# NikolaZubic/2dimageto3dmodel

Measured on NVIDIA H100. Metric: render+loss+GAN images/sec (cfg3: cfg2 render+loss at batch 32 + conv-GAN 256x256 G/D iteration, 1 G : 2 D, Adam), higher is better.
Workload: dtype tf32 (convs) / f32

## Files before the change

2dimageto3dmodel_b200/csrc/b3d_core.cu:

```cuda
#include <atomic>
#include <stdarg.h>
#include <string.h>

#include "b3d_common.cuh"

namespace b3d {
static thread_local char g_err[512] = "";
static thread_local char g_variant[256] = "";
static std::atomic<uint64_t> g_launches{0};

void set_error(const char* fmt, ...) {
    va_list ap;
    va_start(ap, fmt);
    vsnprintf(g_err, sizeof(g_err), fmt, ap);
    va_end(ap);
}
void clear_variant() { g_variant[0] = 0; }
void add_variant(const char* fmt, ...) {
    size_t n = strlen(g_variant);
    if (n + 2 >= sizeof(g_variant)) return;
    if (n) g_variant[n++] = ';';
    va_list ap;
    va_start(ap, fmt);
    vsnprintf(g_variant + n, sizeof(g_variant) - n, fmt, ap);
    va_end(ap);
}
void count_launch(int n) { g_launches.fetch_add((uint64_t)n, std::memory_order_relaxed); }
}

extern "C" {
const char* b3d_last_error(void) { return b3d::g_err; }
const char* b3d_last_variant(void) { return b3d::g_variant; }
int b3d_version(void) { return 420; }
uint64_t b3d_launch_count(void) { return b3d::g_launches.load(std::memory_order_relaxed); }
}
```

2dimageto3dmodel_b200/csrc/tc_conv.cu:

```cuda
#include "tc_common.cuh"

namespace {

constexpr int BM = 128;
constexpr int BK = 32;
constexpr int MMA_K = 8;
constexpr int MAX_TAPS = 25;
constexpr int NTHREADS = 384;

struct ConvParams {
    int N, Hout, Wout, Cout;
    int BW, BH, BI;
    int tiles_x, tiles_y;
    int xbase;
    int ntaps, kslices;
    int sy, sx;
    int dy[MAX_TAPS], dx[MAX_TAPS];
    int wtap[MAX_TAPS];
    int OH, OW, OC, osy, osx;
    float leaky;
    double* stats;
    int fold;
    int fold_y0;
    int mask;
// ... 174 lines not shown
        tc::tma_prefetch_desc(&tmap_w);
        if (p.mask) tc::tma_prefetch_desc(&tmap_m);
        for (int s = 0; s < STAGES; ++s) {
            for (int o = 0; o < OWNERS; ++o) tc::mbar_init(full + o * STAGES + s, 1);
            tc::mbar_init(empty + s, kEmptyArrivals<BN>);
        }
        tc::fence_barrier_init();
    }
    __syncthreads();
    const int KI = p.ntaps / KW * p.kslices;
    const int MS = p.mask ? BN / 32 : 0;
    const int wg = threadIdx.x >> 7;

    if (wg == 0) {
        tc::setmaxnreg_dec<PRODUCER_REGS>();
        if (threadIdx.x == 0) {
            uint32_t git = 0;
            for (int w = blockIdx.x, k = 0; w < work_items; w += gridDim.x, ++k) {
                uint64_t* fb = full + (COOP ? 0 : (k & 1) * STAGES);
                const int cls = w % p.ncls, wq = w / p.ncls, tb = cls * p.ntaps;
                int t = wq % tiles;
                const int c0 = (wq / tiles) * BN;
                const int x0 = p.xbase + (t % p.tiles_x) * p.BW;
                t /= p.tiles_x;
                const int y0 = (t % p.tiles_y) * p.BH, n0 = (t / p.tiles_y) * p.BI;
                for (int it = 0; it < KI; ++it, ++git) {
                    const int s = git % STAGES;
                    tc::mbar_wait(empty + s, ((git / STAGES) & 1) ^ 1);
                    const int tap = it / p.kslices * KW, ks = it % p.kslices;
                    unsigned char* a = base + s * S::STAGE_BYTES;
                    tc::mbar_arrive_expect_tx(fb + s, S::TX_BYTES);
                    if (KW > 1)
                        tc::tma_load_4d(a, &tmap_x, fb + s, ks * BK, x0 + p.dx0, y0 + p.dy[tb + tap], n0);
                    else if (p.fold)
                        tc::tma_load_4d(a, &tmap_x, fb + s, 0, x0 + p.dx[tb + tap], y0 + p.fold_y0 + 4 * ks, n0);
                    else
                        tc::tma_load_4d(a, &tmap_x, fb + s, ks * BK, p.sx * x0 + p.dx[tb + tap], p.sy * y0 + p.dy[tb + tap], n0);
                    tc::tma_load_3d(a + S::A_BYTES, &tmap_w, fb + s, ks * BK, c0, p.wtap[tb + tap]);
                }
                const int mx = p.osx * x0 + p.coox[cls], my = p.osy * y0 + p.cooy[cls];
                for (int m = 0; m < MS; ++m, ++git) {
                    const int s = git % STAGES;
                    tc::mbar_wait(empty + s, ((git / STAGES) & 1) ^ 1);
                    tc::mbar_arrive_expect_tx(fb + s, MASK_BYTES);
                    tc::tma_load_4d(base + s * S::STAGE_BYTES, &tmap_m, fb + s, c0 + mask_chunk_channel(m, G), mx, my, n0);
                }
            }
        }
        return;
    }
    tc::setmaxnreg_inc<CONSUMER_REGS>();

    const int h = wg - 1, tid = threadIdx.x & 127, lane = tid & 31;
    float acc[kBlocks<BN>][BM / 2];
#pragma unroll
    for (int m = 0; m < kBlocks<BN>; ++m)
#pragma unroll
        for (int i = 0; i < BM / 2; ++i) acc[m][i] = 0.f;
    uint32_t git = 0, phase = 0;
    const uint32_t ring = tc::smem_u32(base);
    TileAt at;
    at.lbw = __ffs(p.BW) - 1;
    at.lbwh = at.lbw + __ffs(p.BH) - 1;
    uint64_t* fb = full + (COOP ? 0 : h * STAGES);
    const int cb = COOP ? 128 * h : 0;
    const int cw = (tid >> 5) * 16 + (lane >> 2);
    const int mine = (COOP ? 2 * h : 0) + (tid >> 6);
    for (int k = COOP ? 0 : h;; k += COOP ? 1 : 2) {
        const int w = blockIdx.x + k * gridDim.x;
        if (w >= work_items) break;
        git = (uint32_t)k * (KI + MS);
        const int wq = w / p.ncls, tile = wq % tiles, c0 = (wq / tiles) * BN + cb;
        tile_origin(p, at, tile, w % p.ncls);
        if (KW == 1 && p.fold) mainloop<BN, STAGES, KW, true>(acc, base, fb, empty, KI, git, phase, cb, tid == 0, p.shift);
        else mainloop<BN, STAGES, KW, false>(acc, base, fb, empty, KI, git, phase, cb, tid == 0, p.shift);
        uint32_t neg[kBlocks<BN>][2] = {};
        if (p.mask) {
#pragma unroll
            for (int m = 0; m < kBlocks<BN>; ++m, git += G) {
                uint32_t mstage = 0;
#pragma unroll
                for (int i = 0; i < G; ++i) {
                    const int s = (git + i) % STAGES;
                    tc::mbar_wait(fb + s, (phase >> s) & 1);
                    phase ^= 1u << s;
                    if (i == mine) mstage = ring + s * S::STAGE_BYTES;
                }
                mask_bits<G, STAGES>(neg[m], mstage, cw, lane, empty, git);
            }
        }
#pragma unroll
        for (int m = 0; m < kBlocks<BN>; ++m) {
            if (p.mask) epilogue_block<true>(acc[m], neg[m], p, at, bias, out, c0 + 64 * m, cw, lane);
            else epilogue_block<false>(acc[m], neg[m], p, at, bias, out, c0 + 64 * m, cw, lane);
        }
    }
}

struct WgradParams {
    int N, Hout, Wout, Cout, Cin;
    int BWk, BHk;
    int kx, ky;
    int kh, kw, pad_y, st;
    int xoff;
    int splits;
    int tapmajor;
    int tstep;
};

template <int BN, int STAGES, int NRAW, int T>
struct WSmem {
    static constexpr int DY_BYTES = BM * BK * 4;
    static constexpr int STAGE_BYTES = T * BN * BK * 4;
    static constexpr int WROWS = T == 1 ? 32 : 36;
    static constexpr int RAW_X = (BN / 32) * WROWS * 128;
    static constexpr int RAW_BYTES = (DY_BYTES + RAW_X + 1023) / 1024 * 1024;
    static constexpr int TOTAL = STAGES * STAGE_BYTES + NRAW * RAW_BYTES + 1024 + 256;
};

__host__ __device__ constexpr int wgrad_row_co(int m) { return (m & 35) | ((m & 8) >> 1) | ((m & 16) >> 1) | ((m & 4) << 2); }

__host__ __device__ constexpr int dy_tile_offset(int co, int px) {
    return (co >> 5) * 4096 + px * 128 + ((((co >> 2) & 7) ^ (px & 7)) << 4) + (co & 3) * 4;
}

__host__ __device__ constexpr int xt_chunk(int i) { return (((i & 7) >> 1) ^ ((i >> 4) & 3)) | (((i >> 3) & 1) << 2); }
__host__ __device__ constexpr int xt_src_offset(int i, int px, int wrows) { return ((i >> 6) * wrows + px) * 128 + (i & 7) * 16; }
__host__ __device__ constexpr int xt_dst_offset(int i, int j) {
    return ((i >> 6) * 32 + 4 * (i & 7) + j) * 128 + ((xt_chunk(i) ^ ((4 * (i & 7) + j) & 7)) << 4);
}
template <int BN, int T, int WROWS>
__device__ __forceinline__ void wgrad_transpose(uint32_t src, uint32_t dst, int tid) {
    constexpr int NT = 2 * BN / 128;
    float4 v[NT][T + 3];
#pragma unroll
    for (int n = 0; n < NT; ++n)
#pragma unroll
        for (int u = 0; u < T + 3; ++u) v[n][u] = tc::lds_f32x4(src + xt_src_offset(tid + 128 * n, 4 * xt_chunk(tid + 128 * n) + u, WROWS));
#pragma unroll
    for (int n = 0; n < NT; ++n) {
        const int i = tid + 128 * n;
#pragma unroll
        for (int t = 0; t < T; ++t) {
            const uint32_t d = dst + t * (BN * 128);
            const float4* w = v[n] + t;
            tc::sts_f32x4(d + xt_dst_offset(i, 0), w[0].x, w[1].x, w[2].x, w[3].x);
            tc::sts_f32x4(d + xt_dst_offset(i, 1), w[0].y, w[1].y, w[2].y, w[3].y);
            tc::sts_f32x4(d + xt_dst_offset(i, 2), w[0].z, w[1].z, w[2].z, w[3].z);
            tc::sts_f32x4(d + xt_dst_offset(i, 3), w[0].w, w[1].w, w[2].w, w[3].w);
        }
    }
}

template <int N, int T, int STAGES, int NRAW, int RAW_BYTES, int STAGE_BYTES>
__device__ __forceinline__ void wgrad_consume(float (&acc)[T][N / 2], uint32_t raw_s, uint32_t stage_s, uint64_t* full,
                                              uint64_t* empty, uint64_t* rawfull, uint64_t* rawempty, const int (&aoff)[4],
                                              int first, int step, int KI, int tid, bool zero_first) {
    using Frag = uint32_t[BK / MMA_K][4];
    auto load = [&](Frag& f, int j) {
        const int rb = j % NRAW;
        tc::mbar_wait(rawfull + rb, (j / NRAW) & 1);
#pragma unroll
        for (int k = 0; k < BK / MMA_K; ++k)
#pragma unroll
            for (int e = 0; e < 4; ++e) f[k][e] = tc::lds_u32(raw_s + rb * RAW_BYTES + aoff[e] + k * 1024);
        __syncwarp();
        if ((tid & 31) == 0) tc::mbar_arrive(rawempty + rb);
    };
    auto slice = [&](int j, Frag& f, Frag& g) {
        const int st = j % STAGES;
        tc::mbar_wait(full + st, (j / STAGES) & 1);
        const uint32_t b = stage_s + st * STAGE_BYTES;
        tc::wgmma_fence();
#pragma unroll
        for (int t = 0; t < T; ++t)
#pragma unroll
            for (int k = 0; k < BK / MMA_K; ++k)
                tc::Wgmma<N>::mma_rs(acc[t], f[k], tc::desc_k128(b + t * (N * 128) + k * MMA_K * 4), (zero_first && j == first && k == 0) ? 0u : 1u);
        tc::wgmma_commit();
        tc::wgmma_wait<1>();
#pragma unroll
        for (int k = 0; k < BK / MMA_K; ++k)
#pragma unroll
            for (int e = 0; e < 4; ++e) tc::fence_operand(g[k][e]);
        if (j != first && tid == 0) tc::mbar_arrive(empty + (j - step) % STAGES);
        if (j + step < KI) load(g, j + step);
    };
    Frag f0, f1;
    if (first < KI) load(f0, first);
    for (int j = first; j < KI; j += 2 * step) {
        slice(j, f0, f1);
        if (j + step < KI) slice(j + step, f1, f0);
    }
    tc::wgmma_wait<0>();
#pragma unroll
    for (int k = 0; k < BK / MMA_K; ++k)
#pragma unroll
        for (int e = 0; e < 4; ++e) {
            tc::fence_operand(f0[k][e]);
            tc::fence_operand(f1[k][e]);
        }
#pragma unroll
    for (int t = 0; t < T; ++t)
#pragma unroll
        for (int i = 0; i < N / 2; ++i) tc::fence_operand(acc[t][i]);
    if (first < KI && tid == 0) tc::mbar_arrive(empty + (first + (KI - 1 - first) / step * step) % STAGES);
}

template <int BN, int STAGES, int NRAW, int T>
__global__ void __launch_bounds__(NTHREADS, 1)
wgrad_wgmma_kernel(const __grid_constant__ CUtensorMap tmap_dy, const __grid_constant__ CUtensorMap tmap_x,
                   const WgradParams p, float* __restrict__ dw) {
    using S = WSmem<BN, STAGES, NRAW, T>;
    extern __shared__ unsigned char smem_raw[];
    unsigned char* base = reinterpret_cast<unsigned char*>((reinterpret_cast<uintptr_t>(smem_raw) + 1023) & ~uintptr_t(1023));
    unsigned char* raw = base + STAGES * S::STAGE_BYTES;
    uint64_t* full = reinterpret_cast<uint64_t*>(raw + NRAW * S::RAW_BYTES);
    uint64_t* empty = full + STAGES;
    uint64_t* rawfull = empty + STAGES;
    uint64_t* rawempty = rawfull + NRAW;

    const int co0 = blockIdx.x * BM, ci0 = blockIdx.y * BN;
    const int gpr = p.kw / T;
    const int groups = p.kh * gpr;
    const int grp = blockIdx.z % groups, split = blockIdx.z / groups;
    const int r = grp / gpr, s = grp % gpr;
    const int per_img = p.kx * p.ky;
    const long long ktotal = (long long)p.N * per_img;
    const long long k_lo = ktotal * split / p.splits, k_hi = ktotal * (split + 1) / p.splits;
    const int KI = (int)(k_hi - k_lo);
    const int nact = co0 + 64 < p.Cout ? 2 : 1;

    if (threadIdx.x == 0) {
        tc::tma_prefetch_desc(&tmap_dy);
        tc::tma_prefetch_desc(&tmap_x);
        for (int i = 0; i < STAGES; ++i) {
            tc::mbar_init(full + i, 128);
            tc::mbar_init(empty + i, nact);
        }
        for (int i = 0; i < NRAW; ++i) {
            tc::mbar_init(rawfull + i, 1);
            tc::mbar_init(rawempty + i, 4 * nact);
        }
        tc::fence_barrier_init();
    }
    __syncthreads();
    const int wg = threadIdx.x >> 7, tid = threadIdx.x & 127;

    if (wg == 0) {
        tc::setmaxnreg_dec<80>();
        auto issue = [&](int j) {
            if (tid != 0) return;
            const long long k = k_lo + j;
            const int n = (int)(k / per_img), rem = (int)(k % per_img);
            const int x0 = (rem % p.kx) * p.BWk, y0 = (rem / p.kx) * p.BHk;
            const int rb = j % NRAW;
            unsigned char* dst = raw + rb * S::RAW_BYTES;
            tc::mbar_wait(rawempty + rb, ((j / NRAW) & 1) ^ 1);
            tc::mbar_arrive_expect_tx(rawfull + rb, S::DY_BYTES + S::RAW_X);
            tc::tma_load_5d(dst, &tmap_dy, rawfull + rb, 0, x0, y0, n, co0 / 32);
            tc::tma_load_5d(dst + S::DY_BYTES, &tmap_x, rawfull + rb, 0, p.st * x0 + s + p.xoff, p.st * y0 + r - p.pad_y, n, ci0 / 32);
        };
        for (int j = 0; j < NRAW - 1 && j < KI; ++j) issue(j);
        const uint32_t raw_s = tc::smem_u32(raw), base_s = tc::smem_u32(base);
        for (int it = 0; it < KI; ++it) {
            if (it + NRAW - 1 < KI) issue(it + NRAW - 1);
            const int rb = it % NRAW, st = it % STAGES;
            tc::mbar_wait(rawfull + rb, (it / NRAW) & 1);
            tc::mbar_wait(empty + st, ((it / STAGES) & 1) ^ 1);
            wgrad_transpose<BN, T, S::WROWS>(raw_s + rb * S::RAW_BYTES + S::DY_BYTES, base_s + st * S::STAGE_BYTES, tid);
            tc::fence_proxy_async();
            tc::mbar_arrive(full + st);
            tc::named_sync(2, 128);
        }
        return;
    }
    tc::setmaxnreg_inc<208>();

    const int h = wg - 1, lane = tid & 31;
    if (h >= nact) return;
    int aoff[4];
#pragma unroll
    for (int e = 0; e < 4; ++e)
        aoff[e] = dy_tile_offset(h * 64 + wgrad_row_co((tid >> 5) * 16 + (lane >> 2) + 8 * (e & 1)), (lane & 3) + 4 * (e >> 1));
    float acc[T][BN / 2];
#pragma unroll
    for (int t = 0; t < T; ++t)
#pragma unroll
        for (int i = 0; i < BN / 2; ++i) acc[t][i] = 0.f;
    wgrad_consume<BN, T, STAGES, NRAW, S::RAW_BYTES, S::STAGE_BYTES>(acc, tc::smem_u32(raw), tc::smem_u32(base), full, empty, rawfull,
                                                                     rawempty, aoff, 0, 1, KI, tid, true);
    if (KI == 0) return;
    const int m_a = (tid >> 5) * 16 + (lane >> 2);
    const int cq = ci0 + 2 * (lane & 3);
#pragma unroll
    for (int t = 0; t < T; ++t) {
        const int sc = s + t * p.tstep;
#pragma unroll
        for (int e = 0; e < 2; ++e) {
            const int co = co0 + h * 64 + wgrad_row_co(m_a + 8 * e);
            if (co >= p.Cout) continue;
#pragma unroll
            for (int j = 0; j < BN / 8; ++j) {
                const int ci = cq + 8 * j;
                if (ci >= p.Cin) continue;
                const float v0 = acc[t][4 * j + 2 * e], v1 = acc[t][4 * j + 2 * e + 1];
                if (p.tapmajor) {
                    atomicAdd(reinterpret_cast<float2*>(dw + ((size_t)(r * p.kw + sc) * p.Cout + co) * p.Cin + ci), make_float2(v0, v1));
                } else {
                    atomicAdd(dw + (((size_t)co * p.Cin + ci) * p.kh + r) * p.kw + sc, v0);
                    atomicAdd(dw + (((size_t)co * p.Cin + ci + 1) * p.kh + r) * p.kw + sc, v1);
                }
            }
        }
    }
}

template <int BN, int STAGES, int NRAW, int T>
int launch_wgrad(const CUtensorMap& mdy, const CUtensorMap& mx, const WgradParams& p, float* dw, dim3 grid, cudaStream_t st) {
    using S = WSmem<BN, STAGES, NRAW, T>;
    static_assert(S::TOTAL <= 227 * 1024, "wgrad pipeline does not fit shared memory");
    B3D_CUDA_OK(cudaFuncSetAttribute(wgrad_wgmma_kernel<BN, STAGES, NRAW, T>, cudaFuncAttributeMaxDynamicSharedMemorySize, S::TOTAL));
    wgrad_wgmma_kernel<BN, STAGES, NRAW, T><<<grid, NTHREADS, S::TOTAL, st>>>(mdy, mx, p, dw);
    B3D_LAUNCH_OK();
    b3d::add_variant("wgrad_wgmma<%d,%d,%d,%d>", BN, STAGES, NRAW, T);
    return B3D_OK;
}

constexpr int STEM_KW = 5, STEM_STAGES = 4, STEM_NRAW = 3;
constexpr int STEM_BATCH = 3;
struct StemSmem {
    static constexpr int DY_BYTES = 64 * BK * 4;
    static constexpr int WPX = BK + STEM_KW - 1;
    static constexpr int RAW_X_MAX = 8 * WPX * 32;
    static constexpr int RAW_BYTES = (DY_BYTES + RAW_X_MAX + 1023) / 1024 * 1024;
    static constexpr int TILE_BYTES = 64 * BK * 4;
    static constexpr int STAGE_BYTES = STEM_KW * TILE_BYTES;
    static constexpr int TOTAL = STEM_STAGES * STAGE_BYTES + STEM_NRAW * RAW_BYTES + 1024 + 256;
};

__global__ void __launch_bounds__(NTHREADS, 1)
wgrad_stem_kernel(const __grid_constant__ CUtensorMap tmap_dy, const __grid_constant__ CUtensorMap tmap_x,
                  const WgradParams p, int fold_kh, float* __restrict__ dw) {
    using S = StemSmem;
    extern __shared__ unsigned char smem_raw[];
    unsigned char* base = reinterpret_cast<unsigned char*>((reinterpret_cast<uintptr_t>(smem_raw) + 1023) & ~uintptr_t(1023));
    unsigned char* raw = base + STEM_STAGES * S::STAGE_BYTES;
    uint64_t* full = reinterpret_cast<uint64_t*>(raw + STEM_NRAW * S::RAW_BYTES);
    uint64_t* empty = full + STEM_STAGES;
    uint64_t* rawfull = empty + STEM_STAGES;
    uint64_t* rawempty = rawfull + STEM_NRAW;

    const int co0 = blockIdx.x * 64, split = blockIdx.y;
    const int per_img = p.kx * p.ky;
    const long long ktotal = (long long)p.N * per_img;
    const long long k_lo = ktotal * split / p.splits, k_hi = ktotal * (split + 1) / p.splits;
    const int KI = (int)(k_hi - k_lo);
    const int creal = 8 * fold_kh;
    const int xbytes = fold_kh * S::WPX * 32;

    if (threadIdx.x == 0) {
        tc::tma_prefetch_desc(&tmap_dy);
        tc::tma_prefetch_desc(&tmap_x);
        for (int i = 0; i < STEM_STAGES; ++i) {
            tc::mbar_init(full + i, 128);
            tc::mbar_init(empty + i, 1);
        }
        for (int i = 0; i < STEM_NRAW; ++i) {
            tc::mbar_init(rawfull + i, 1);
            tc::mbar_init(rawempty + i, 4);
        }
        tc::fence_barrier_init();
    }
    __syncthreads();
    const int wg = threadIdx.x >> 7, tid = threadIdx.x & 127;

    if (wg == 0) {
        tc::setmaxnreg_dec<56>();
        auto issue = [&](int j) {
            if (tid != 0) return;
            const long long k = k_lo + j;
            const int n = (int)(k / per_img), rem = (int)(k % per_img);
            const int x0 = (rem % p.kx) * BK, y0 = rem / p.kx;
            const int rb = j % STEM_NRAW;
            unsigned char* dst = raw + rb * S::RAW_BYTES;
            tc::mbar_wait(rawempty + rb, ((j / STEM_NRAW) & 1) ^ 1);
            tc::mbar_arrive_expect_tx(rawfull + rb, S::DY_BYTES + xbytes);
            tc::tma_load_5d(dst, &tmap_dy, rawfull + rb, 0, x0, y0, n, co0 / 32);
            tc::tma_load_4d(dst + S::DY_BYTES, &tmap_x, rawfull + rb, 0, x0, y0 - p.pad_y, n);
        };
        for (int i = tid; i < STEM_STAGES * STEM_KW * (64 - creal) * 8; i += 128) {
            const int c = creal + (i >> 3) % (64 - creal), tile = (i >> 3) / (64 - creal);
            *reinterpret_cast<float4*>(base + tile * S::TILE_BYTES + c * 128 + (i & 7) * 16) = make_float4(0.f, 0.f, 0.f, 0.f);
        }
        for (int j = 0; j < STEM_NRAW - 1 && j < KI; ++j) issue(j);
        const int ntask = fold_kh * 8 * STEM_KW * 8;
        const uint32_t raw_s = tc::smem_u32(raw), base_s = tc::smem_u32(base);
        for (int it = 0; it < KI; ++it) {
            if (it + STEM_NRAW - 1 < KI) issue(it + STEM_NRAW - 1);
            const int rb = it % STEM_NRAW, st = it % STEM_STAGES;
            tc::mbar_wait(rawfull + rb, (it / STEM_NRAW) & 1);
            tc::mbar_wait(empty + st, ((it / STEM_STAGES) & 1) ^ 1);
            const uint32_t src = raw_s + rb * S::RAW_BYTES + S::DY_BYTES;
            const uint32_t dst = base_s + st * S::STAGE_BYTES;
            for (int i0 = tid; i0 < ntask; i0 += STEM_BATCH * 128) {
                float v[STEM_BATCH][4];
                uint32_t d[STEM_BATCH];
#pragma unroll
                for (int g = 0; g < STEM_BATCH; ++g) {
                    const int i = i0 + 128 * g;
                    if (i >= ntask) break;
                    const int ci = i & 7, u = i >> 3;
                    const int s = u % STEM_KW, q = (u / STEM_KW) & 7, r = u / (STEM_KW * 8);
                    const uint32_t a = src + ((r * S::WPX + 4 * q + s) * 8 + ci) * 4;
#pragma unroll
                    for (int e = 0; e < 4; ++e) v[g][e] = tc::lds_f32(a + 32 * e);
                    d[g] = dst + s * S::TILE_BYTES + (8 * r + ci) * 128 + ((q ^ ci) << 4);
                }
#pragma unroll
                for (int g = 0; g < STEM_BATCH; ++g) {
                    if (i0 + 128 * g >= ntask) break;
                    tc::sts_f32x4(d[g], v[g][0], v[g][1], v[g][2], v[g][3]);
                }
            }
            tc::fence_proxy_async();
            tc::mbar_arrive(full + st);
            tc::named_sync(2, 128);
        }
        return;
    }
    tc::setmaxnreg_inc<224>();

    const int h = wg - 1, lane = tid & 31;
    int aoff[4];
#pragma unroll
    for (int e = 0; e < 4; ++e)
        aoff[e] = dy_tile_offset(wgrad_row_co((tid >> 5) * 16 + (lane >> 2) + 8 * (e & 1)), (lane & 3) + 4 * (e >> 1));
    float acc[STEM_KW][32];
#pragma unroll
    for (int t = 0; t < STEM_KW; ++t)
#pragma unroll
        for (int i = 0; i < 32; ++i) acc[t][i] = 0.f;
    static_assert(S::TILE_BYTES == 64 * 128, "a tap's B tile is 64 channel rows of 128 bytes");
    wgrad_consume<64, STEM_KW, STEM_STAGES, STEM_NRAW, S::RAW_BYTES, S::STAGE_BYTES>(acc, tc::smem_u32(raw), tc::smem_u32(base), full, empty,
                                                                                     rawfull, rawempty, aoff, h, 2, KI, tid, false);
    if (h >= KI) return;
    const int m_a = (tid >> 5) * 16 + (lane >> 2);
#pragma unroll
    for (int t = 0; t < STEM_KW; ++t) {
#pragma unroll
        for (int e = 0; e < 2; ++e) {
            const int co = co0 + wgrad_row_co(m_a + 8 * e);
#pragma unroll
            for (int j = 0; j < 8; ++j) {
                const int ci = 8 * j + 2 * (lane & 3);
                if (ci >= creal) continue;
                const float v0 = acc[t][4 * j + 2 * e], v1 = acc[t][4 * j + 2 * e + 1];
                if (p.tapmajor) {
                    atomicAdd(reinterpret_cast<float2*>(dw + ((size_t)t * p.Cout + co) * p.Cin + ci), make_float2(v0, v1));
                } else {
                    atomicAdd(dw + ((size_t)co * p.Cin + ci) * STEM_KW + t, v0);
                    atomicAdd(dw + ((size_t)co * p.Cin + ci + 1) * STEM_KW + t, v1);
                }
            }
        }
    }
}

int wgrad_splits(int base_ctas, long long ktotal) {
    constexpr long long FIXED = 16;
    const long long sms = tc::num_sms();
    long long smax = ktotal / 8;
    if (smax > 8 * sms) smax = 8 * sms;
    int best = 1;
    long long best_cost = -1;
    for (long long s = 1; s <= smax; ++s) {
        const long long cost = (base_ctas * s + sms - 1) / sms * ((ktotal + s - 1) / s + FIXED);
        if (best_cost < 0 || cost < best_cost) { best = (int)s; best_cost = cost; }
    }
    return best;
}

template <int BN, int STAGES, int KW = 1>
int launch_conv(const CUtensorMap& mx, const CUtensorMap& mw, const CUtensorMap& mm, const ConvParams& p, const float* bias, float* out,
                int tiles, cudaStream_t st) {
    using S = CSmem<BN, STAGES, KW>;
    static_assert(S::TOTAL <= 227 * 1024, "conv pipeline does not fit shared memory");
    B3D_CUDA_OK(cudaFuncSetAttribute(conv_wgmma_kernel<BN, STAGES, KW>, cudaFuncAttributeMaxDynamicSharedMemorySize, S::TOTAL));
    const int work = tiles * b3d::ceil_div(p.Cout, BN) * p.ncls;
    const int sms = tc::num_sms();
    conv_wgmma_kernel<BN, STAGES, KW><<<work < sms ? work : sms, NTHREADS, S::TOTAL, st>>>(mx, mw, mm, p, bias, out, tiles, work);
    B3D_LAUNCH_OK();
    if (KW > 1) b3d::add_variant("conv_wgmma_rowwin<%d,%d,%d>", BN, KW, STAGES);
    else b3d::add_variant("conv_wgmma<%d,%d>", BN, STAGES);
    return B3D_OK;
}

template <int BN>
int launch_rowwin(int kw, const CUtensorMap& mx, const CUtensorMap& mw, const CUtensorMap& mm, const ConvParams& p, const float* bias,
                  float* out, int tiles, cudaStream_t st) {
    if (kw == 2) return launch_conv<BN, BN == 64 ? 5 : 4, 2>(mx, mw, mm, p, bias, out, tiles, st);
    if (kw == 3) return launch_conv<BN, BN == 64 ? 4 : 3, 3>(mx, mw, mm, p, bias, out, tiles, st);
    return launch_conv<BN, BN == 64 ? 3 : 2, 5>(mx, mw, mm, p, bias, out, tiles, st);
}

int pow2_floor(int v) {
    int p = 1;
    while (p * 2 <= v) p *= 2;
    return p;
}

}

extern "C" {

int b3d_conv2d_tf32(const float* x, const float* wt, const float* bias, float* out, int N, int H, int W, int Cin,
                    int Hout, int Wout, int Cout, int ntaps, const int* dy, const int* dx, int sy, int sx, int OH,
                    int OW, int OC, int osy, int osx, int ooy, int oox, float leaky, const int* wtap,
                    int wtaps_total, double* stats, int fold_kh, int fold_pad, const b3d_conv_opts* opts, void* stream) {
    B3D_REQUIRE(N > 0 && H > 0 && W > 0 && Hout > 0 && Wout > 0 && Cout > 0, B3D_EINVAL, "b3d_conv2d_tf32: bad sizes");
    B3D_REQUIRE(Cin > 0 && Cin % BK == 0, B3D_EINVAL, "b3d_conv2d_tf32: Cin=%d must be a multiple of %d", Cin, BK);
    B3D_REQUIRE(ntaps >= 1 && ntaps <= MAX_TAPS && dy && dx, B3D_EINVAL, "b3d_conv2d_tf32: bad taps");
    B3D_REQUIRE(x && wt && out, B3D_EINVAL, "b3d_conv2d_tf32: null pointer");
    B3D_REQUIRE(sy >= 1 && sy <= 2 && sx >= 1 && sx <= 2, B3D_EINVAL, "b3d_conv2d_tf32: stride must be 1 or 2");
    if (!wtap) wtaps_total = ntaps;
    B3D_REQUIRE(wtaps_total >= ntaps || wtap, B3D_EINVAL, "b3d_conv2d_tf32: bad weight tap count");
    for (int t = 0; wtap && t < ntaps; ++t)
        B3D_REQUIRE(wtap[t] >= 0 && wtap[t] < wtaps_total, B3D_EINVAL, "b3d_conv2d_tf32: weight tap %d out of range", wtap[t]);
    B3D_CHECK_ALIGNED(x);
    B3D_CHECK_ALIGNED(wt);
    b3d::clear_variant();

    const float* mask = opts ? opts->mask : nullptr;
    const float mslope = opts ? opts->mask_slope : 1.f;
    B3D_REQUIRE(!mask || (reinterpret_cast<uintptr_t>(mask) % 16 == 0 && OC % 4 == 0), B3D_EINVAL,
                "b3d_conv2d_tf32: the mask needs a 16-byte aligned base and OC %% 4 == 0 (OC=%d)", OC);
    const int stats_sum = (opts && opts->stats_sum_only) ? 1 : 0;
    const int xpitch = (opts && opts->x_row_pitch) ? opts->x_row_pitch : W;
    const int ncls = (opts && opts->nclass > 1) ? opts->nclass : 1;
    B3D_REQUIRE(ncls <= 4 && ntaps % ncls == 0 && (ncls == 1 || (sy == 1 && sx == 1 && fold_kh == 0)), B3D_EINVAL,
                "b3d_conv2d_tf32: nclass=%d needs <= 4 equal tap groups of a stride-1 launch", ncls);
    const int tpc = ntaps / ncls;
    int cooy[4] = {ooy, ooy, ooy, ooy}, coox[4] = {oox, oox, oox, oox};
    for (int c = 0; c < ncls && ncls > 1; ++c) { cooy[c] = opts->class_ooy[c]; coox[c] = opts->class_oox[c]; }
    B3D_REQUIRE(xpitch >= W && (fold_kh == 0 || xpitch == W), B3D_EINVAL, "b3d_conv2d_tf32: x_row_pitch=%d must be >= W=%d (and absent with the on-the-fly fold)", xpitch, W);
    if (fold_kh > 0) {
        B3D_REQUIRE(fold_kh <= 8 && Cin == 32 * ((8 * fold_kh + 31) / 32) && sy == 1 && sx == 1 && !wtap && Wout % BM == 0,
                    B3D_EINVAL, "b3d_conv2d_tf32: on-the-fly fold needs 8 input channels, stride 1 and Wout %% 128 == 0 (Wout=%d)", Wout);
    }
    B3D_REQUIRE(!stats || mask || (osy == 1 && osx == 1), B3D_EINVAL, "b3d_conv2d_tf32: statistics need a dense output");
    const bool bn256 = Cout % 256 == 0 && (long long)N * Hout * Wout / BM * (Cout / 256) * ncls >= tc::num_sms();
    const int BN = bn256 ? 256 : Cout > 64 ? 128 : 64;
    cudaStream_t st = (cudaStream_t)stream;
    CUtensorMap mw;
    {
        const uint64_t dims[3] = {(uint64_t)Cin, (uint64_t)Cout, (uint64_t)wtaps_total};
        const uint64_t strides[2] = {(uint64_t)Cin * 4, (uint64_t)Cout * Cin * 4};
        const uint32_t box[3] = {(uint32_t)BK, (uint32_t)BN, 1};
        if (int rc = tc::make_tmap_f32(&mw, wt, 3, dims, strides, box)) return rc;
    }

    int g_kw = 0, g_step = 1, g_wstep = 1;
    if (sy == 1 && sx == 1 && fold_kh == 0) {
        int kw_ = 1;
        while (kw_ < tpc && dy[kw_] == dy[0]) ++kw_;
        const int step = kw_ > 1 ? dx[1] - dx[0] : 1;
        const int wstep = (wtap && kw_ > 1) ? wtap[1] - wtap[0] : 1;
        bool grid_ok = tpc % kw_ == 0 && (kw_ == 2 || kw_ == 3 || kw_ == 5) && (step == 1 || step == -1) && wstep >= 1 && wstep <= 2 &&
                       (ncls == 1 || wtap != nullptr);
        for (int t = 0; grid_ok && t < ntaps; ++t) {
            const int tc_ = t % tpc, t0 = t - tc_;
            grid_ok = dy[t] == dy[t0 + (tc_ / kw_) * kw_] && dx[t] == dx[0] + (tc_ % kw_) * step;
            if (wtap) grid_ok = grid_ok && wtap[t] == wtap[t0 + (tc_ / kw_) * kw_] + (tc_ % kw_) * wstep;
        }
        if (grid_ok && BN <= 128) { g_kw = kw_; g_step = step; g_wstep = wstep; }
    }

    auto run = [&](int xlo, int xhi) -> int {
        const int wspan = xhi - xlo;
        ConvParams p{};
        p.N = N; p.Hout = Hout; p.Wout = xhi; p.Cout = Cout; p.xbase = xlo;
        p.BW = pow2_floor(wspan < BM ? wspan : BM);
        p.BH = pow2_floor(Hout < BM / p.BW ? Hout : BM / p.BW);
        p.BI = BM / (p.BW * p.BH);
        p.tiles_x = b3d::ceil_div(wspan, p.BW);
        p.tiles_y = b3d::ceil_div(Hout, p.BH);
        const int tiles = p.tiles_x * p.tiles_y * b3d::ceil_div(N, p.BI);
        p.ntaps = tpc; p.kslices = Cin / BK; p.sy = sy; p.sx = sx; p.ncls = ncls;
        for (int t = 0; t < ntaps; ++t) { p.dy[t] = dy[t]; p.dx[t] = dx[t]; p.wtap[t] = wtap ? wtap[t] : t; }
        for (int c = 0; c < 4; ++c) { p.cooy[c] = cooy[c]; p.coox[c] = coox[c]; }
        p.OH = OH; p.OW = OW; p.OC = OC; p.osy = osy; p.osx = osx;
        p.leaky = leaky;
        p.stats = stats;
        p.mask = mask != nullptr; p.mslope = mslope; p.stats_sum = stats_sum;
        p.fold = fold_kh; p.fold_y0 = -fold_pad;
        {
            const unsigned long long esn = p.BI > 1 ? (unsigned long long)OH * OW * OC : 0, esy = p.BH > 1 ? (unsigned long long)osy * OW * OC : 0,
                                     esx = (unsigned long long)osx * OC;
            B3D_REQUIRE((p.BI - 1) * esn + (p.BH - 1) * esy + (p.BW - 1) * esx + OC < (1ull << 32), B3D_EINVAL,
                        "b3d_conv2d_tf32: a %d x %d x %d pixel tile spans more than 2^32 elements of the output", p.BI, p.BH, p.BW);
            p.esn = (uint32_t)esn; p.esy = (uint32_t)esy; p.esx = (uint32_t)esx;
        }
        CUtensorMap mm{};
        if (mask) {
            const uint64_t dims[4] = {(uint64_t)OC, (uint64_t)OW, (uint64_t)OH, (uint64_t)N};
            const uint64_t strides[3] = {(uint64_t)OC * 4, (uint64_t)OW * OC * 4, (uint64_t)OH * OW * OC * 4};
            const uint32_t box[4] = {(uint32_t)BK, (uint32_t)(osx * (p.BW - 1) + 1), (uint32_t)(osy * (p.BH - 1) + 1), (uint32_t)p.BI};
            const uint32_t es[4] = {1, (uint32_t)osx, (uint32_t)osy, 1};
            if (int rc = tc::make_tmap_f32(&mm, mask, 4, dims, strides, box, es)) return rc;
        }
        CUtensorMap mx;
        if (g_kw && wspan >= BM) {
            p.dx0 = g_step > 0 ? dx[0] : dx[g_kw - 1];
            for (int t = 0; t < g_kw; ++t) p.shift[t] = dx[t] - p.dx0;
            const uint64_t dims[4] = {(uint64_t)Cin, (uint64_t)W, (uint64_t)H, (uint64_t)N};
            const uint64_t strides[3] = {(uint64_t)Cin * 4, (uint64_t)xpitch * Cin * 4, (uint64_t)H * xpitch * Cin * 4};
            const uint32_t box[4] = {(uint32_t)BK, (uint32_t)(BM + g_kw - 1), 1, 1};
            if (int rc = tc::make_tmap_f32(&mx, x, 4, dims, strides, box)) return rc;
            CUtensorMap mwr;
// ... 122 lines not shown
```

Before: 1441.

## Restructure stem wgrad: transpose dy once, read shifted x taps as A fragments

The stem weight-gradient kernel no longer builds five tap-shifted copies of the input tile per stage. The producer now transposes only the dy tile into one B tile. The consumers load the tap-shifted x windows directly from the raw TMA buffer as register A fragments, one set per tap. The taps are split across the two consumer warpgroups (3 and 2 taps), where before the K iterations were interleaved between them. This cuts shared-memory transpose traffic and stage size, in exchange for more A-fragment register loads, uneven tap work between the warpgroups, and shuffle-based paired atomics in the epilogue.

```diff
diff --git a/2dimageto3dmodel_b200/csrc/b3d_core.cu b/2dimageto3dmodel_b200/csrc/b3d_core.cu
--- a/2dimageto3dmodel_b200/csrc/b3d_core.cu
+++ b/2dimageto3dmodel_b200/csrc/b3d_core.cu
@@ -31,6 +31,6 @@
 extern "C" {
 const char* b3d_last_error(void) { return b3d::g_err; }
 const char* b3d_last_variant(void) { return b3d::g_variant; }
-int b3d_version(void) { return 420; }
+int b3d_version(void) { return 430; }
 uint64_t b3d_launch_count(void) { return b3d::g_launches.load(std::memory_order_relaxed); }
 }
diff --git a/2dimageto3dmodel_b200/csrc/tc_conv.cu b/2dimageto3dmodel_b200/csrc/tc_conv.cu
--- a/2dimageto3dmodel_b200/csrc/tc_conv.cu
+++ b/2dimageto3dmodel_b200/csrc/tc_conv.cu
@@ -350,18 +350,34 @@
     }
 }
 
-template <int N, int T, int STAGES, int NRAW, int RAW_BYTES, int STAGE_BYTES>
+__host__ __device__ constexpr int dyt_src_offset(int i, int u) {
+    return dy_tile_offset(32 * (i >> 6) + 4 * (i & 7), 4 * xt_chunk(i) + u);
+}
+__device__ __forceinline__ void dy_transpose(uint32_t src, uint32_t dst, int tid) {
+    float4 v[4];
+#pragma unroll
+    for (int u = 0; u < 4; ++u) v[u] = tc::lds_f32x4(src + dyt_src_offset(tid, u));
+    tc::sts_f32x4(dst + xt_dst_offset(tid, 0), v[0].x, v[1].x, v[2].x, v[3].x);
+    tc::sts_f32x4(dst + xt_dst_offset(tid, 1), v[0].y, v[1].y, v[2].y, v[3].y);
+    tc::sts_f32x4(dst + xt_dst_offset(tid, 2), v[0].z, v[1].z, v[2].z, v[3].z);
+    tc::sts_f32x4(dst + xt_dst_offset(tid, 3), v[0].w, v[1].w, v[2].w, v[3].w);
+}
+
+template <int N, int T, int TA, int STAGES, int NRAW, int RAW_BYTES, int STAGE_BYTES, int KSTEP = 1024>
 __device__ __forceinline__ void wgrad_consume(float (&acc)[T][N / 2], uint32_t raw_s, uint32_t stage_s, uint64_t* full,
-                                              uint64_t* empty, uint64_t* rawfull, uint64_t* rawempty, const int (&aoff)[4],
+                                              uint64_t* empty, uint64_t* rawfull, uint64_t* rawempty, const int (&aoff)[TA][4],
                                               int first, int step, int KI, int tid, bool zero_first) {
-    using Frag = uint32_t[BK / MMA_K][4];
+    static_assert(TA == 1 || TA == T, "one A fragment set for all taps, or one per tap");
+    using Frag = uint32_t[TA][BK / MMA_K][4];
     auto load = [&](Frag& f, int j) {
         const int rb = j % NRAW;
         tc::mbar_wait(rawfull + rb, (j / NRAW) & 1);
 #pragma unroll
-        for (int k = 0; k < BK / MMA_K; ++k)
-#pragma unroll
-            for (int e = 0; e < 4; ++e) f[k][e] = tc::lds_u32(raw_s + rb * RAW_BYTES + aoff[e] + k * 1024);
+        for (int a = 0; a < TA; ++a)
+#pragma unroll
+            for (int k = 0; k < BK / MMA_K; ++k)
+#pragma unroll
+                for (int e = 0; e < 4; ++e) f[a][k][e] = tc::lds_u32(raw_s + rb * RAW_BYTES + aoff[a][e] + k * KSTEP);
         __syncwarp();
         if ((tid & 31) == 0) tc::mbar_arrive(rawempty + rb);
     };
@@ -374,13 +390,16 @@
         for (int t = 0; t < T; ++t)
 #pragma unroll
             for (int k = 0; k < BK / MMA_K; ++k)
-                tc::Wgmma<N>::mma_rs(acc[t], f[k], tc::desc_k128(b + t * (N * 128) + k * MMA_K * 4), (zero_first && j == first && k == 0) ? 0u : 1u);
+                tc::Wgmma<N>::mma_rs(acc[t], f[TA == 1 ? 0 : t][k], tc::desc_k128(b + (TA == 1 ? t * (N * 128) : 0) + k * MMA_K * 4),
+                                     (zero_first && j == first && k == 0) ? 0u : 1u);
         tc::wgmma_commit();
         tc::wgmma_wait<1>();
 #pragma unroll
-        for (int k = 0; k < BK / MMA_K; ++k)
-#pragma unroll
-            for (int e = 0; e < 4; ++e) tc::fence_operand(g[k][e]);
+        for (int a = 0; a < TA; ++a)
+#pragma unroll
+            for (int k = 0; k < BK / MMA_K; ++k)
+#pragma unroll
+                for (int e = 0; e < 4; ++e) tc::fence_operand(g[a][k][e]);
         if (j != first && tid == 0) tc::mbar_arrive(empty + (j - step) % STAGES);
         if (j + step < KI) load(g, j + step);
     };
@@ -392,12 +411,14 @@
     }
     tc::wgmma_wait<0>();
 #pragma unroll
-    for (int k = 0; k < BK / MMA_K; ++k)
-#pragma unroll
-        for (int e = 0; e < 4; ++e) {
-            tc::fence_operand(f0[k][e]);
-            tc::fence_operand(f1[k][e]);
-        }
+    for (int a = 0; a < TA; ++a)
+#pragma unroll
+        for (int k = 0; k < BK / MMA_K; ++k)
+#pragma unroll
+            for (int e = 0; e < 4; ++e) {
+                tc::fence_operand(f0[a][k][e]);
+                tc::fence_operand(f1[a][k][e]);
+            }
 #pragma unroll
     for (int t = 0; t < T; ++t)
 #pragma unroll
@@ -477,17 +498,17 @@
 
     const int h = wg - 1, lane = tid & 31;
     if (h >= nact) return;
-    int aoff[4];
+    int aoff[1][4];
 #pragma unroll
     for (int e = 0; e < 4; ++e)
-        aoff[e] = dy_tile_offset(h * 64 + wgrad_row_co((tid >> 5) * 16 + (lane >> 2) + 8 * (e & 1)), (lane & 3) + 4 * (e >> 1));
+        aoff[0][e] = dy_tile_offset(h * 64 + wgrad_row_co((tid >> 5) * 16 + (lane >> 2) + 8 * (e & 1)), (lane & 3) + 4 * (e >> 1));
     float acc[T][BN / 2];
 #pragma unroll
     for (int t = 0; t < T; ++t)
 #pragma unroll
         for (int i = 0; i < BN / 2; ++i) acc[t][i] = 0.f;
-    wgrad_consume<BN, T, STAGES, NRAW, S::RAW_BYTES, S::STAGE_BYTES>(acc, tc::smem_u32(raw), tc::smem_u32(base), full, empty, rawfull,
-                                                                     rawempty, aoff, 0, 1, KI, tid, true);
+    wgrad_consume<BN, T, 1, STAGES, NRAW, S::RAW_BYTES, S::STAGE_BYTES>(acc, tc::smem_u32(raw), tc::smem_u32(base), full, empty, rawfull,
+                                                                        rawempty, aoff, 0, 1, KI, tid, true);
     if (KI == 0) return;
     const int m_a = (tid >> 5) * 16 + (lane >> 2);
     const int cq = ci0 + 2 * (lane & 3);
@@ -526,16 +547,60 @@
 }
 
 constexpr int STEM_KW = 5, STEM_STAGES = 4, STEM_NRAW = 3;
-constexpr int STEM_BATCH = 3;
 struct StemSmem {
     static constexpr int DY_BYTES = 64 * BK * 4;
     static constexpr int WPX = BK + STEM_KW - 1;
     static constexpr int RAW_X_MAX = 8 * WPX * 32;
     static constexpr int RAW_BYTES = (DY_BYTES + RAW_X_MAX + 1023) / 1024 * 1024;
-    static constexpr int TILE_BYTES = 64 * BK * 4;
-    static constexpr int STAGE_BYTES = STEM_KW * TILE_BYTES;
+    static constexpr int STAGE_BYTES = 64 * BK * 4;
     static constexpr int TOTAL = STEM_STAGES * STAGE_BYTES + STEM_NRAW * RAW_BYTES + 1024 + 256;
 };
+
+template <int S0, int T>
+__device__ __forceinline__ void stem_consume_taps(const WgradParams& p, int creal, int co0, uint32_t raw_s, uint32_t stage_s,
+                                                  uint64_t* full, uint64_t* empty, uint64_t* rawfull, uint64_t* rawempty, int KI,
+                                                  int tid, float* __restrict__ dw) {
+    using S = StemSmem;
+    const int lane = tid & 31, m_a = (tid >> 5) * 16 + (lane >> 2);
+    int aoff[T][4];
+#pragma unroll
+    for (int t = 0; t < T; ++t)
+#pragma unroll
+        for (int e = 0; e < 4; ++e) {
+            const int m = m_a + 8 * (e & 1);
+            aoff[t][e] = S::DY_BYTES + (((m >> 3) * S::WPX + (lane & 3) + 4 * (e >> 1) + S0 + t) * 8 + (m & 7)) * 4;
+        }
+    float acc[T][32];
+#pragma unroll
+    for (int t = 0; t < T; ++t)
+#pragma unroll
+        for (int i = 0; i < 32; ++i) acc[t][i] = 0.f;
+    wgrad_consume<64, T, T, STEM_STAGES, STEM_NRAW, S::RAW_BYTES, S::STAGE_BYTES, 8 * 32>(acc, raw_s, stage_s, full, empty, rawfull,
+                                                                                          rawempty, aoff, 0, 1, KI, tid, true);
+    if (KI == 0) return;
+    const bool odd = lane & 4;
+#pragma unroll
+    for (int t = 0; t < T; ++t) {
+#pragma unroll
+        for (int e = 0; e < 2; ++e) {
+            const int cf = m_a + 8 * e;
+            if (cf >= creal) continue;
+#pragma unroll
+            for (int j = 0; j < 8; ++j) {
+                const int co = co0 + 8 * j + 2 * (lane & 3);
+                const float v0 = acc[t][4 * j + 2 * e], v1 = acc[t][4 * j + 2 * e + 1];
+                if (p.tapmajor) {
+                    const float other = __shfl_xor_sync(0xffffffffu, odd ? v0 : v1, 4);
+                    atomicAdd(reinterpret_cast<float2*>(dw + ((size_t)(S0 + t) * p.Cout + co + odd) * p.Cin + (cf & ~1)),
+                              odd ? make_float2(other, v1) : make_float2(v0, other));
+                } else {
+                    atomicAdd(dw + ((size_t)co * p.Cin + cf) * STEM_KW + S0 + t, v0);
+                    atomicAdd(dw + ((size_t)(co + 1) * p.Cin + cf) * STEM_KW + S0 + t, v1);
+                }
+            }
+        }
+    }
+}
 
 __global__ void __launch_bounds__(NTHREADS, 1)
 wgrad_stem_kernel(const __grid_constant__ CUtensorMap tmap_dy, const __grid_constant__ CUtensorMap tmap_x,
@@ -562,13 +627,17 @@
         tc::tma_prefetch_desc(&tmap_x);
         for (int i = 0; i < STEM_STAGES; ++i) {
             tc::mbar_init(full + i, 128);
-            tc::mbar_init(empty + i, 1);
+            tc::mbar_init(empty + i, 2);
         }
         for (int i = 0; i < STEM_NRAW; ++i) {
             tc::mbar_init(rawfull + i, 1);
-            tc::mbar_init(rawempty + i, 4);
+            tc::mbar_init(rawempty + i, 8);
         }
         tc::fence_barrier_init();
+    }
+    for (int i = threadIdx.x; i < STEM_NRAW * (S::RAW_X_MAX - xbytes) / 16; i += NTHREADS) {
+        const int slot = i / ((S::RAW_X_MAX - xbytes) / 16), o = i % ((S::RAW_X_MAX - xbytes) / 16);
+        *reinterpret_cast<float4*>(raw + slot * S::RAW_BYTES + S::DY_BYTES + xbytes + 16 * o) = make_float4(0.f, 0.f, 0.f, 0.f);
     }
     __syncthreads();
     const int wg = threadIdx.x >> 7, tid = threadIdx.x & 127;
@@ -587,40 +656,14 @@
             tc::tma_load_5d(dst, &tmap_dy, rawfull + rb, 0, x0, y0, n, co0 / 32);
             tc::tma_load_4d(dst + S::DY_BYTES, &tmap_x, rawfull + rb, 0, x0, y0 - p.pad_y, n);
         };
-        for (int i = tid; i < STEM_STAGES * STEM_KW * (64 - creal) * 8; i += 128) {
-            const int c = creal + (i >> 3) % (64 - creal), tile = (i >> 3) / (64 - creal);
-            *reinterpret_cast<float4*>(base + tile * S::TILE_BYTES + c * 128 + (i & 7) * 16) = make_float4(0.f, 0.f, 0.f, 0.f);
-        }
         for (int j = 0; j < STEM_NRAW - 1 && j < KI; ++j) issue(j);
-        const int ntask = fold_kh * 8 * STEM_KW * 8;
         const uint32_t raw_s = tc::smem_u32(raw), base_s = tc::smem_u32(base);
         for (int it = 0; it < KI; ++it) {
             if (it + STEM_NRAW - 1 < KI) issue(it + STEM_NRAW - 1);
             const int rb = it % STEM_NRAW, st = it % STEM_STAGES;
             tc::mbar_wait(rawfull + rb, (it / STEM_NRAW) & 1);
             tc::mbar_wait(empty + st, ((it / STEM_STAGES) & 1) ^ 1);
-            const uint32_t src = raw_s + rb * S::RAW_BYTES + S::DY_BYTES;
-            const uint32_t dst = base_s + st * S::STAGE_BYTES;
-            for (int i0 = tid; i0 < ntask; i0 += STEM_BATCH * 128) {
-                float v[STEM_BATCH][4];
-                uint32_t d[STEM_BATCH];
-#pragma unroll
-                for (int g = 0; g < STEM_BATCH; ++g) {
-                    const int i = i0 + 128 * g;
-                    if (i >= ntask) break;
-                    const int ci = i & 7, u = i >> 3;
-                    const int s = u % STEM_KW, q = (u / STEM_KW) & 7, r = u / (STEM_KW * 8);
-                    const uint32_t a = src + ((r * S::WPX + 4 * q + s) * 8 + ci) * 4;
-#pragma unroll
-                    for (int e = 0; e < 4; ++e) v[g][e] = tc::lds_f32(a + 32 * e);
-                    d[g] = dst + s * S::TILE_BYTES + (8 * r + ci) * 128 + ((q ^ ci) << 4);
-                }
-#pragma unroll
-                for (int g = 0; g < STEM_BATCH; ++g) {
-                    if (i0 + 128 * g >= ntask) break;
-                    tc::sts_f32x4(d[g], v[g][0], v[g][1], v[g][2], v[g][3]);
-                }
-            }
+            dy_transpose(raw_s + rb * S::RAW_BYTES, base_s + st * S::STAGE_BYTES, tid);
             tc::fence_proxy_async();
             tc::mbar_arrive(full + st);
             tc::named_sync(2, 128);
@@ -628,41 +671,9 @@
         return;
     }
     tc::setmaxnreg_inc<224>();
-
-    const int h = wg - 1, lane = tid & 31;
-    int aoff[4];
-#pragma unroll
-    for (int e = 0; e < 4; ++e)
-        aoff[e] = dy_tile_offset(wgrad_row_co((tid >> 5) * 16 + (lane >> 2) + 8 * (e & 1)), (lane & 3) + 4 * (e >> 1));
-    float acc[STEM_KW][32];
-#pragma unroll
-    for (int t = 0; t < STEM_KW; ++t)
-#pragma unroll
-        for (int i = 0; i < 32; ++i) acc[t][i] = 0.f;
-    static_assert(S::TILE_BYTES == 64 * 128, "a tap's B tile is 64 channel rows of 128 bytes");
-    wgrad_consume<64, STEM_KW, STEM_STAGES, STEM_NRAW, S::RAW_BYTES, S::STAGE_BYTES>(acc, tc::smem_u32(raw), tc::smem_u32(base), full, empty,
-                                                                                     rawfull, rawempty, aoff, h, 2, KI, tid, false);
-    if (h >= KI) return;
-    const int m_a = (tid >> 5) * 16 + (lane >> 2);
-#pragma unroll
-    for (int t = 0; t < STEM_KW; ++t) {
-#pragma unroll
-        for (int e = 0; e < 2; ++e) {
-            const int co = co0 + wgrad_row_co(m_a + 8 * e);
-#pragma unroll
-            for (int j = 0; j < 8; ++j) {
-                const int ci = 8 * j + 2 * (lane & 3);
-                if (ci >= creal) continue;
-                const float v0 = acc[t][4 * j + 2 * e], v1 = acc[t][4 * j + 2 * e + 1];
-                if (p.tapmajor) {
-                    atomicAdd(reinterpret_cast<float2*>(dw + ((size_t)t * p.Cout + co) * p.Cin + ci), make_float2(v0, v1));
-                } else {
-                    atomicAdd(dw + ((size_t)co * p.Cin + ci) * STEM_KW + t, v0);
-                    atomicAdd(dw + ((size_t)co * p.Cin + ci + 1) * STEM_KW + t, v1);
-                }
-            }
-        }
-    }
+    const uint32_t raw_s = tc::smem_u32(raw), base_s = tc::smem_u32(base);
+    if (wg == 1) stem_consume_taps<0, 3>(p, creal, co0, raw_s, base_s, full, empty, rawfull, rawempty, KI, tid, dw);
+    else stem_consume_taps<3, 2>(p, creal, co0, raw_s, base_s, full, empty, rawfull, rawempty, KI, tid, dw);
 }
 
 int wgrad_splits(int base_ctas, long long ktotal) {
```

Result: faster. 1476 (median of 6 runs) (+2.4%).
